# rayanirban/DiffSplitting

Measured on AMD Instinct MI355X. Metric: sampled images/sec (2000-step 128x128 SR3), higher is better.
Workload: dtype bf16; 1 GPU; sr_sr3_16_128: GaussianDiffusion.p_sample_loop, 16->128 SR3 UNet (97.8M params), T=2000 linear schedule; one step = UNet forward + posterior update of the batch; batch_per_gpu=16, global_batch=16, image=128x128x3, sample_steps=2000, parallelism=1 independent replicas, final RCCL all-gather, hipgraph=True, streams=1, noise=device Philox4x32-10, weights=random-init, seed 0

## Files before the change

diffsplitting_amd/csrc/dsx_conv_direct.hip:

```cpp
#include "dsx_conv_common.h"

namespace dsx {

template <typename DT>
__global__ __launch_bounds__(256) void k_conv_first(const ConvArgs a) {
  constexpr bool F32 = sizeof(DT) == 4;
  constexpr int ES = (int)sizeof(DT);
  constexpr int KSTEP = F32 ? 2 : 16;
  constexpr int NS16 = 4;
  __shared__ __attribute__((aligned(16))) unsigned char sm[18 * 18 * 7 * 4 + 64 * 4];
  DT* patch = (DT*)sm;
  int* kofft = (int*)(sm + 18 * 18 * 7 * 4);

  const int tid = threadIdx.x, lane = tid & 63;
  const int wave = __builtin_amdgcn_readfirstlane(tid >> 6);
  const int li = lane & 31, lh = lane >> 5;
  const int Cin = a.C0 + a.C1, K = 9 * Cin;
  const int tiles_x = a.Wo >> 4, tiles_y = a.Ho >> 4;
  const int t = blockIdx.x % (tiles_x * tiles_y), b = blockIdx.x / (tiles_x * tiles_y);
  const int ty = t / tiles_x, tx = t - ty * tiles_x;
  const int oy0 = ty * 16, ox0 = tx * 16;
  const int NBLK = (a.Cout + 31) >> 5;

  for (int e = tid; e < 18 * 18 * Cin; e += 256) {
// ... 37 lines not shown
#pragma unroll
  for (int mb = 0; mb < 2; ++mb)
#pragma unroll
    for (int nb = 0; nb < 2; ++nb)
#pragma unroll
      for (int r = 0; r < 16; ++r) acc[mb][nb][r] = 0.f;

#pragma unroll
  for (int mb = 0; mb < 2; ++mb) {
    const int m = (wave * 2 + mb) * 32 + li;
    const int base = ((m >> 4) * 18 + (m & 15)) * Cin;
    if constexpr (F32) {
      const int nsteps = (K + 1) >> 1;
      const float* wp = (const float*)a.wpack;
      for (int s = 0; s < nsteps; ++s) {
        const float pv = ((const float*)patch)[base + kofft[2 * s + lh]];
#pragma unroll
        for (int nb = 0; nb < 2; ++nb) {
          if (nb < NBLK) acc[mb][nb] = __builtin_amdgcn_mfma_f32_32x32x2f32(wp[(nb * 32 + s) * 64 + lane], pv, acc[mb][nb], 0, 0, 0);
        }
      }
    } else {
      const unsigned char* pb = (const unsigned char*)patch + base * 2;
#pragma unroll
      for (int s = 0; s < NS16; ++s) {
        unsigned w4[4];
#pragma unroll
        for (int q = 0; q < 4; ++q) {
          const unsigned lo = *(const unsigned short*)(pb + koff[s * 8 + 2 * q]);
          const unsigned hi = *(const unsigned short*)(pb + koff[s * 8 + 2 * q + 1]);
          w4[q] = lo | (hi << 16);
        }
        const f32x4_t px = __builtin_bit_cast(f32x4_t, make_uint4(w4[0], w4[1], w4[2], w4[3]));
#pragma unroll
        for (int nb = 0; nb < 2; ++nb)
          if (nb < NBLK) acc[mb][nb] = mfma_step<DT>(wf[nb * NS16 + s], px, acc[mb][nb]);
      }
    }
  }
  (void)KSTEP; (void)ES;

  const int okind = a.out_bf16;
#pragma unroll
  for (int nb = 0; nb < 2; ++nb) {
    const int nbase = nb * 32 + 16 * lh;
    if (nb >= NBLK) continue;
    float s1[16], s2[16];
#pragma unroll
    for (int r = 0; r < 16; ++r) { s1[r] = 0.f; s2[r] = 0.f; }
    const bool live = nbase < a.Cout;
#pragma unroll
    for (int mb = 0; mb < 2; ++mb) {
      const int m = (wave * 2 + mb) * 32 + li;
      const size_t opix = ((size_t)b * a.Ho + (oy0 + (m >> 4))) * a.Wo + (ox0 + (m & 15));
      float x[16], pv[16];
#pragma unroll
      for (int r = 0; r < 16; ++r) { x[r] = acc[mb][nb][r]; pv[r] = 0.f; }
      if (live) {
        if (a.bias) {
#pragma unroll
          for (int j = 0; j < 4; ++j) { const float4 tt = *(const float4*)(a.bias + nbase + 4 * j); pv[4 * j] = tt.x; pv[4 * j + 1] = tt.y; pv[4 * j + 2] = tt.z; pv[4 * j + 3] = tt.w; }
#pragma unroll
          for (int r = 0; r < 16; ++r) x[r] += pv[r];
        }
        store16<true>(a.out, opix * a.out_ld + nbase, x, okind, 16);
#pragma unroll
        for (int r = 0; r < 16; ++r) { const float d = x[r] - pv[r]; s1[r] += d; s2[r] += d * d; }
      }
    }
    if (a.stat_part != nullptr) {
      float w1 = row16_fold(s1, lane), w2 = row16_fold(s2, lane);
      w1 += __shfl_xor(w1, 16, 64);
      w2 += __shfl_xor(w2, 16, 64);
      const int nch = tiles_x * tiles_y * 4, chunk = t * 4 + wave;
      const int n = nbase + row16_fold_reg(li);
      if (li < 16 && n < a.Cout) {
        float* pp = a.stat_part + (((size_t)b * nch + chunk) * a.Cout + n) * 2;
        pp[0] = w1; pp[1] = w2;
      }
    }
  }
}

bool conv_first_applicable(int ks, int stride, const ConvArgs& a, bool gn) {
  const int C = a.C0 + a.C1;
  return ks == 3 && stride == 1 && !a.up && !gn && !a.swish && C >= 1 && C <= 7 && a.Cout >= 16 && a.Cout <= 64 &&
         (a.Cout & 15) == 0 && (a.Ho & 15) == 0 && (a.Wo & 15) == 0 && a.Ho == a.Hs && a.Wo == a.Ws && a.out_ld == a.Cout;
}
hipError_t launch_conv_first(int dtype, const ConvArgs& a, hipStream_t st) {
  const unsigned grid = (unsigned)(a.B * (a.Ho >> 4) * (a.Wo >> 4));
  if (dtype == 1) hipLaunchKernelGGL(k_conv_first<__bf16>, dim3(grid), dim3(256), 0, st, a);
  else if (dtype == 2) hipLaunchKernelGGL(k_conv_first<_Float16>, dim3(grid), dim3(256), 0, st, a);
  else hipLaunchKernelGGL(k_conv_first<float>, dim3(grid), dim3(256), 0, st, a);
  return hipGetLastError();
}

__global__ void k_conv_naive(const NaiveConvArgs na) {
  const ConvArgs& a = na.c;
  const long long total = (long long)a.B * a.Ho * a.Wo * a.Cout;
  const int C = a.C0 + a.C1;
  const int pad = na.ks / 2;
  const int Hi = a.up ? a.Hs * 2 : a.Hs, Wi = a.up ? a.Ws * 2 : a.Ws;
  for (long long idx = blockIdx.x * (long long)blockDim.x + threadIdx.x; idx < total;
       idx += (long long)gridDim.x * blockDim.x) {
    const int n = (int)(idx % a.Cout);
    long long p = idx / a.Cout;
    const int ox = (int)(p % a.Wo); p /= a.Wo;
    const int oy = (int)(p % a.Ho);
    const int b = (int)(p / a.Ho);
    float acc = 0.f;
    for (int dy = 0; dy < na.ks; ++dy) {
      const int iy = oy * na.stride + dy - pad;
      if (iy < 0 || iy >= Hi) continue;
      for (int dx = 0; dx < na.ks; ++dx) {
        const int ix = ox * na.stride + dx - pad;
        if (ix < 0 || ix >= Wi) continue;
        const int sy = a.up ? iy >> 1 : iy, sx = a.up ? ix >> 1 : ix;
        const size_t so = ((size_t)b * a.Hs + sy) * a.Ws + sx;
        const float* w = na.w + (((size_t)n * na.ks + dy) * na.ks + dx) * C;
        for (int c = 0; c < C; ++c) {
          float v = c < a.C0 ? act_load_kind(a.src0, so * a.C0 + c, a.act_bf16)
                             : act_load_kind(a.src1, so * a.C1 + (c - a.C0), a.act_bf16);
          if (a.gn_scale) v = v * a.gn_scale[(size_t)b * C + c] + a.gn_shift[(size_t)b * C + c];
          if (a.swish) v = swish_f(v);
          acc = fmaf(v, w[c], acc);
        }
      }
    }
    const size_t opix = ((size_t)b * a.Ho + oy) * a.Wo + ox;
    float v = acc + (a.bias ? a.bias[n] : 0.f);
    if (a.film) v += a.film[(size_t)b * a.film_bs + n];
    if (a.resid) v += act_load_kind(a.resid, opix * a.resid_ld + n, a.act_bf16);
    if (na.sigmoid_out) v = 1.0f / (1.0f + __expf(-v));
    act_store(a.out, opix * a.out_ld + n, v, a.out_bf16);
  }
}

hipError_t launch_conv_naive(const NaiveConvArgs& a, hipStream_t st) {
  const long long total = (long long)a.c.B * a.c.Ho * a.c.Wo * a.c.Cout;
  long long blocks = (total + 255) / 256;
  if (blocks > 8192) blocks = 8192;
  hipLaunchKernelGGL(k_conv_naive, dim3((unsigned)blocks), dim3(256), 0, st, a);
  return hipGetLastError();
}

}
```

diffsplitting_amd/csrc/dsx_kernels.h:

```cpp
#pragma once
#include <hip/hip_runtime.h>
#include <stdint.h>

namespace dsx {

struct PrefetchArgs {
  const void* base;
  unsigned slice_bytes;
  int nslices;
  unsigned* sink;
};
inline unsigned fastdiv_magic(unsigned d) { return d <= 1 ? 0u : (unsigned)((1ull << 32) / d) + 1u; }
#if defined(__HIPCC__)
__device__ __forceinline__ unsigned fastdiv(unsigned n, unsigned magic) { return magic ? __umulhi(n, magic) : n; }
struct PfAcc { unsigned v[4]; };
__device__ __forceinline__ PfAcc l2_prefetch(const PrefetchArgs& pf, unsigned lin_block, unsigned nblocks_total, int tid, int nthreads) {
  PfAcc acc = {{0u, 0u, 0u, 0u}};
  if (pf.base == nullptr || pf.nslices <= 0) return acc;
  const unsigned label = lin_block & 7u, j = lin_block >> 3, n8 = (nblocks_total + 7u) >> 3;
  const unsigned lines = pf.slice_bytes >> 7;
  const unsigned per = (lines + n8 - 1u) / n8, l0 = j * per;
  const unsigned l1 = l0 + per < lines ? l0 + per : lines;
  const int s0 = pf.nslices < 8 ? (int)(label % (unsigned)pf.nslices) : (int)label;
  const int sstep = pf.nslices < 8 ? pf.nslices : 8;
// ... 85 lines not shown
            ps[u] += ch == 0 ? a.count * p : 0.0;
          }
        }
      }
#pragma unroll
      for (int u = 0; u < 8; ++u) { s += ps[u]; q += pq[u]; }
    }
  };
  const int c_own = c_lo + tid;
  const bool own = tid < cpg;
  const float g_own = own ? a.gamma[c_own] : 0.f, b_own = own ? a.beta[c_own] : 0.f;
  if (n0 > 0) accumulate(a.part0, a.f32_0, n0, a.nchunk0, a.C0, c_lo, a.piv0);
  if (n1 > 0) accumulate(a.part1, a.f32_1, n1, a.nchunk1, a.C1, c_lo + n0 - a.C0, a.piv1);
#pragma unroll
  for (int o = 32; o > 0; o >>= 1) { s += __shfl_xor(s, o, 64); q += __shfl_xor(q, o, 64); }
  if constexpr (NW > 1) {
    if ((tid & 63) == 0) { red[2 * (tid >> 6)] = s; red[2 * (tid >> 6) + 1] = q; }
    __syncthreads();
    s = 0; q = 0;
#pragma unroll
    for (int w = 0; w < NW; ++w) { s += red[2 * w]; q += red[2 * w + 1]; }
  }
  const double n = a.count * cpg;
  const double mean = s / n;
  double var = q / n - mean * mean;
  if (var < 0) var = 0;
  const float rstd = (float)(1.0 / sqrt(var + (double)a.eps));
  const float meanf = (float)mean;
  if (own) {
    const float sc = rstd * g_own;
    a.scale[(size_t)b * C + c_own] = sc;
    a.shift[(size_t)b * C + c_own] = b_own - meanf * sc;
  }
  for (int c = c_lo + tid + NT; c < c_lo + cpg; c += NT) {
    const float sc = rstd * a.gamma[c];
    a.scale[(size_t)b * C + c] = sc;
    a.shift[(size_t)b * C + c] = a.beta[c] - meanf * sc;
  }
}
#endif

struct ConvArgs {
  const void* src0;
  const void* src1;
  int act_bf16;
  int out_bf16;
  int C0, C1;
  int B, Hs, Ws;
  int up;
  int Ho, Wo;
  const float* gn_scale;
  const float* gn_shift;
  int has_gn;
  int swish;
  int stage_mode;
  const void* wpack;
  const float* bias;
  const float* film;
  int film_bs;
  const void* resid;
  int resid_ld;
  void* out;
  int out_ld;
  int Cout;
  int nblocks;
  int kchunks;
  int tw_log2, th_log2, tb_log2;
  int tiles_x, tiles_y, m_tiles, n_tiles;
  int lds_row;
  int cpg;
  int ws_wg_per_n;
  int ws_cpg;
  int xcd_bands;
  int ws_map;
  int ws_nt_log2;
  int ws_per;
  int ws_adv_x, ws_adv_y, ws_adv_b;
  int ws_dpy, ws_dpx;
  unsigned mg_tiles_x, mg_per_img, mg_pw, mg_wpn, mg_per;
  int ws_bigdiv;
  float* stat_part;
  unsigned* handoff_timeouts;
  int ws_direct;
  unsigned long long* stamp;
  int stamp_block;
  int ablate;
  const void* gn_part0; int gn_nchunk0, gn_pf32_0;
  const void* gn_part1; int gn_nchunk1, gn_pf32_1;
  StatPivot gn_piv0, gn_piv1;
  const float* gn_gamma; const float* gn_beta;
  int gn_groups; float gn_eps;
  PrefetchArgs pf;
  int fin_on;
  GnFinArgs fin;
  int ksplit;
  int groups_per_split;
  long long slab_stride;
};

enum ConvTile { TILE_256x128 = 0, TILE_128x128, TILE_64x128, TILE_256x64, TILE_128x64, TILE_64x64, TILE_128x32, TILE_256x32, TILE_COUNT };
struct ConvTileInfo { int BM, BN, WM; bool fuses_stats; };
ConvTileInfo conv_tile_info(int tile, bool ws = false);
int conv_chunk_multiple(int ks);
constexpr int conv_lds_row(int ks, int stride, int tw_log2, int cpg) {
  const int pixb = 64 * cpg + 16;
  const int pw = ((1 << tw_log2) - 1) * stride + ks;
  int rb = (pw * pixb + 15) & ~15;
  if (ks == 1 || stride != 1) return rb;
  if (tw_log2 == 4) rb = (rb + 255) & ~255;
  else if (tw_log2 == 3) { rb = (rb + 127) & ~127; if (((rb >> 7) & 1) == 0) rb += 128; }
  return rb;
}
size_t conv_lds_bytes(int dtype, int tile, int ks, int stride, const ConvArgs& a);
hipError_t launch_conv(int dtype, int tile, int ks, int stride, const ConvArgs& a, hipStream_t st);
size_t conv_ws_lds_bytes(int dtype, int tile, int ks, const ConvArgs& a);
hipError_t launch_conv_ws(int dtype, int tile, int ks, const ConvArgs& a, hipStream_t st);
bool conv_img_applicable(int dtype, int ks, int stride, const ConvArgs& a, bool gn, int gn_groups);
hipError_t launch_conv_img(int dtype, int ks, const ConvArgs& a, hipStream_t st);
bool conv_first_applicable(int ks, int stride, const ConvArgs& a, bool gn);
hipError_t launch_conv_first(int dtype, const ConvArgs& a, hipStream_t st);
hipError_t conv_init();
hipError_t ops_init();

struct NaiveConvArgs {
  ConvArgs c;
  const float* w;
  int ks, stride;
  int sigmoid_out;
};
hipError_t launch_conv_naive(const NaiveConvArgs& a, hipStream_t st);

hipError_t launch_chan_stats(const void* x, int bf16, int B, int HW, int C, int nchunk, double* part,
                             hipStream_t st);
hipError_t launch_gn_finalize(const GnFinArgs& a, hipStream_t st);

struct TembArgs {
  int flavour;
  int B;
  int n_time;
  const float* time;
  const float* table;
  const int* step_ctr;
  int per_sample;
  int inner;
  const float* freq;
  const float* w1; const float* b1;
  const float* w2; const float* b2;
  const float* wf; const float* bf;
  int F;
  float* film;
};
hipError_t launch_temb(const TembArgs& a, hipStream_t st);

struct SplitKReduceArgs {
  const float* slab; int nsplit; long long slab_stride;
  long long M; int N; int HW;
  const float* bias; const float* film; int film_bs;
  const void* resid; int resid_ld;
  void* out;
  int act_bf16;
  float* stat_part;
};
hipError_t launch_splitk_reduce(const SplitKReduceArgs& a, hipStream_t st);

struct AttnArgs {
  const void* q; const void* k; const void* v; int ld;
  void* out; int ldo;
  int storage;
  int B, L, C;
  float div, inv_div;
};
bool attn_supported(int C, int L);
hipError_t launch_attn(const AttnArgs& a, bool col_split, hipStream_t st);

hipError_t launch_nchw_slice_to_nhwc(const float* src, void* dst, int dst_bf16, int B, int C, int ctot, int coff,
                                     int HW, hipStream_t st);
hipError_t launch_nhwc_to_nchw(const float* src, float* dst, int B, int C, int H, int W, hipStream_t st);

constexpr int kUpdateCols = 7;
struct UpdateArgs {
  float* x;
  void* x_act;
  int x_act_kind;
  const float* net;
  float* x0_hist;
  int use_noise;
  const unsigned long long* loop_params;
  const float* tab;
  int n_steps;
  const int* step_ctr;
  int predict_eps, clip;
  int per_sample;
  int B, C, H, W;
  const unsigned long long* sample_ids;
};
hipError_t launch_update(const UpdateArgs& a, hipStream_t st);
constexpr int kStreamRows = 32;
struct StreamIds { unsigned long long subseq[kStreamRows]; };
template <class F>
static inline hipError_t each_stream_chunk(int B, const uint64_t* ids, uint64_t draw, F&& f) {
  for (int b0 = 0; b0 < B; b0 += kStreamRows) {
    StreamIds s{};
// ... 323 lines not shown
```

diffsplitting_amd/csrc/dsx_plan.cpp:

```cpp
#include "dsx_rt.h"

static std::vector<int> tile_order(const char* e, const std::vector<int>& dflt) {
  if (!*e) return dflt;
  std::vector<int> v;
  for (const char* p = e; *p;) {
    v.push_back(atoi(p));
    while (*p && *p != ',') ++p;
    if (*p == ',') ++p;
  }
  return v;
}

PlanKnobs dsx::read_plan_knobs() {
  PlanKnobs k;
  static const struct { const char* name; int PlanKnobs::*field; } ints[] = {
      {"DSX_FIRST", &PlanKnobs::first}, {"DSX_IMG", &PlanKnobs::img}, {"DSX_WS", &PlanKnobs::ws},
      {"DSX_WS_1X1", &PlanKnobs::ws_1x1}, {"DSX_WS_MIN_GRID", &PlanKnobs::ws_min_grid}, {"DSX_WS_G2", &PlanKnobs::ws_g2},
      {"DSX_WS_G2_MIN64", &PlanKnobs::ws_g2_min64}, {"DSX_WS_G2_MIN128", &PlanKnobs::ws_g2_min128},
      {"DSX_WS_G4_MIN64", &PlanKnobs::ws_g4_min64}, {"DSX_WS_C4", &PlanKnobs::ws_c4},
      {"DSX_WS_C4_MIN", &PlanKnobs::ws_c4_min}, {"DSX_WS_DIRECT", &PlanKnobs::ws_direct}, {"DSX_WS_MAP3", &PlanKnobs::ws_map3},
      {"DSX_XCD_BANDS", &PlanKnobs::xcd_bands}, {"DSX_HOST_FIN", &PlanKnobs::host_fin},
      {"DSX_PREFETCH", &PlanKnobs::prefetch}, {"DSX_PREFETCH_WS", &PlanKnobs::prefetch_ws},
      {"DSX_FUSE_STATS", &PlanKnobs::fuse_stats}, {"DSX_NARROW_G2", &PlanKnobs::narrow_g2},
      {"DSX_MIN_GRID", &PlanKnobs::min_grid}, {"DSX_SPLITK", &PlanKnobs::splitk}, {"DSX_ATTN_CS", &PlanKnobs::attn_cs},
#ifdef DSX_DIAG
      {"DSX_ABLATE", &PlanKnobs::ablate},
#endif
  };
  static const struct { const char* name; std::vector<int> PlanKnobs::*field; } lists[] = {
      {"DSX_TILES_WIDE", &PlanKnobs::tiles_wide}, {"DSX_TILES_NARROW", &PlanKnobs::tiles_narrow},
      {"DSX_TILES_SLIM", &PlanKnobs::tiles_slim}, {"DSX_TILES_WIDE_SPLIT", &PlanKnobs::tiles_wide_split},
      {"DSX_TILES_NARROW_SPLIT", &PlanKnobs::tiles_narrow_split}, {"DSX_TILES_NARROW_G2", &PlanKnobs::tiles_narrow_g2},
      {"DSX_TILES_WS_WIDE", &PlanKnobs::tiles_ws_wide}, {"DSX_TILES_WS_WIDE_1X1", &PlanKnobs::tiles_ws_wide_1x1},
      {"DSX_TILES_WS_WIDE_1X1_RAW", &PlanKnobs::tiles_ws_wide_1x1_raw}, {"DSX_TILES_WS_NARROW", &PlanKnobs::tiles_ws_narrow},
  };
  for (const auto& e : ints)
    if (const char* v = getenv(e.name)) k.*e.field = atoi(v);
  for (const auto& e : lists)
    if (const char* v = getenv(e.name)) k.*e.field = tile_order(v, k.*e.field);
  const char* impl = getenv("DSX_CONV_IMPL");
  k.conv_naive = impl && !strcmp(impl, "naive");
  if (const char* path = getenv("DSX_PLAN_DUMP")) k.plan_dump = path;
  if (const char* se = getenv("DSX_STAMP_OP")) {
    const char* comma = strchr(se, ',');
    k.stamp_op = atoi(se);
    k.stamp_block = comma ? atoi(comma + 1) : 0;
  }
  return k;
}

hipError_t dsx::launch_op(const PlanOp& o, hipStream_t st) {
  switch (o.launcher) {
    case L_CONV_FIRST: return launch_conv_first(o.dtype, o.args.conv, st);
    case L_CONV_IMG: return launch_conv_img(o.dtype, o.ks, o.args.conv, st);
    case L_CONV_WS: return launch_conv_ws(o.dtype, o.tile, o.ks, o.args.conv, st);
    case L_CONV_MFMA: return launch_conv(o.dtype, o.tile, o.ks, o.stride, o.args.conv, st);
    case L_SPLITK_REDUCE: return launch_splitk_reduce(o.args.reduce, st);
    case L_CONV_NAIVE: return launch_conv_naive(o.args.naive, st);
    case L_CHAN_STATS: {
      const ChanStatsArgs& c = o.args.stats;
      return launch_chan_stats(c.x, c.xbf, c.B, c.HW, c.C, c.nchunk, c.part, st);
    }
    case L_GN_FINALIZE: return launch_gn_finalize(o.args.fin, st);
    case L_ATTN: return launch_attn(o.args.attn, o.col_split != 0, st);
  }
  return hipErrorInvalidValue;
}

static int dump_plan(const dsx_exec* ex) {
  static const struct { const char* name; size_t bytes; } L[] = {
      {"conv_first", sizeof(ConvArgs)}, {"conv_img", sizeof(ConvArgs)}, {"conv_ws", sizeof(ConvArgs)},
      {"conv_mfma", sizeof(ConvArgs)}, {"splitk_reduce", sizeof(SplitKReduceArgs)}, {"conv_naive", sizeof(NaiveConvArgs)},
      {"chan_stats", sizeof(ChanStatsArgs)}, {"gn_finalize", sizeof(GnFinArgs)}, {"attn", sizeof(AttnArgs)}};
  FILE* f = fopen(ex->knobs.plan_dump.c_str(), "w");
  if (!f) return fail(DSX_ERR_INVALID, "DSX_PLAN_DUMP: cannot write %s", ex->knobs.plan_dump.c_str());
  for (size_t i = 0; i < ex->ops.size(); ++i) {
    const PlanOp& o = ex->ops[i];
    const char* name = (o.launcher == L_GN_FINALIZE && gn_finalize_is_wide(o.args.fin)) ? "gn_finalize_wide" : L[o.launcher].name;
    fprintf(f, "%zu kind=%d desc=\"%s\" flops=%.17g bytes=%.17g launcher=%s dtype=%d tile=%d ks=%d stride=%d col_split=%d args=",
            i, o.kind, o.desc.c_str(), o.flops, o.bytes, name, o.dtype, o.tile, o.ks, o.stride, o.col_split);
    const unsigned char* p = (const unsigned char*)&o.args;
    for (size_t b = 0; b < L[o.launcher].bytes; ++b) fprintf(f, "%02x", p[b]);
    fputc('\n', f);
  }
  fclose(f);
  return DSX_OK;
}

static int add_op(dsx_exec* ex, int kind, const std::string& desc, double flops, double bytes, Launcher launcher) {
  PlanOp op;
  op.kind = kind; op.desc = desc; op.flops = flops; op.bytes = bytes; op.launcher = launcher;
  ex->ops.push_back(op);
  return (int)ex->ops.size() - 1;
}
static std::string fmt(const char* f, ...) {
  char buf[256];
  va_list ap;
  va_start(ap, f);
  vsnprintf(buf, sizeof buf, f, ap);
  va_end(ap);
  return buf;
}

static char* ws_alloc(dsx_exec* ex, size_t bytes) {
  size_t off = (ex->ws_used + 255) & ~(size_t)255;
  ex->ws_used = off + bytes;
  if (ex->sizing) return nullptr;
// ... 135 lines not shown
    if (wpn > a.m_tiles) wpn = (a.m_tiles + unit - 1) / unit * unit;
  }
  return wpn;
}

static void decide_ws_chunks(const PlanKnobs& k, int dtype, int ks, int tile, ConvArgs& a) {
  auto take = [&](bool wanted, int cpg) {
    ConvArgs t = a;
    t.ws_cpg = cpg; t.lds_row = conv_lds_row(ks, 1, a.tw_log2, cpg);
    if (wanted && conv_ws_lds_bytes(dtype, tile, ks, t) != 0) { a.ws_cpg = cpg; a.lds_row = t.lds_row; }
  };
  if (ks == 3) {
    const int min_chunks = conv_tile_info(tile).BM == 64 ? k.ws_g2_min64 : k.ws_g2_min128;
    take(k.ws_g2 && a.kchunks >= min_chunks, 2);
    take(k.ws_g2 && a.kchunks >= k.ws_g4_min64, 4);
  }
  if (ks == 1) take(k.ws_c4 && a.kchunks >= k.ws_c4_min, 4);
  if (ks == 1 && k.ws_direct && !a.has_gn && !a.swish) {
    ConvArgs t = a;
    t.ws_direct = 1;
    if (conv_ws_lds_bytes(dtype, tile, ks, t) != 0) a.ws_direct = 1;
  }
}

static int decide_ws_startup(const PlanKnobs& k, int ks, ConvArgs& w) {
  w.xcd_bands = k.xcd_bands;
  w.ws_wg_per_n = ws_wg_per_n(w);
  const bool map3 = k.ws_map3 && ks == 1 && w.n_tiles >= 2 && w.n_tiles <= 32;
  if (map3) {
    int wpn3 = std::max(8, (256 / w.n_tiles) / 8 * 8);
    if (wpn3 > w.m_tiles) wpn3 = (w.m_tiles + 7) / 8 * 8;
    w.ws_wg_per_n = wpn3;
  }
  const int NT = w.n_tiles, wpn = w.ws_wg_per_n, per_img = w.tiles_x * w.tiles_y;
  w.ws_map = map3 ? 3 : ((NT <= 8 && 8 % NT == 0 && wpn % (8 / NT) == 0) ? 0 : ((NT % 8) == 0 ? 1 : 2));
  w.ws_nt_log2 = NT <= 8 ? ilog2(NT) : 0;
  w.ws_per = map3 ? NT : (NT >> 3);
  w.ws_adv_x = wpn % w.tiles_x; w.ws_adv_y = (wpn / w.tiles_x) % w.tiles_y; w.ws_adv_b = wpn / per_img;
  const int PW = ((1 << w.tw_log2) - 1) + ks;
  const int upg = 4 * (w.ws_cpg ? w.ws_cpg : conv_chunk_multiple(ks));
  const int pstep = 256 / upg;
  w.ws_dpy = pstep / PW; w.ws_dpx = pstep - w.ws_dpy * PW;
  w.mg_tiles_x = fastdiv_magic((unsigned)w.tiles_x); w.mg_per_img = fastdiv_magic((unsigned)per_img);
  w.mg_pw = fastdiv_magic((unsigned)PW); w.mg_wpn = fastdiv_magic((unsigned)wpn);
  w.mg_per = fastdiv_magic((unsigned)std::max(1, w.ws_per));
  w.ws_bigdiv = ((long long)w.m_tiles + wpn >= 65536 || w.tiles_x >= 65536 || per_img >= 65536) ? 1 : 0;
  auto exact = [](unsigned d, unsigned magic, unsigned nmax) {
    for (unsigned n = 0; n <= nmax; ++n) {
      const unsigned q = magic ? (unsigned)(((unsigned long long)n * magic) >> 32) : n;
      if (q != n / d) return false;
    }
    return true;
  };
  const unsigned grid = (unsigned)(NT * wpn);
  const unsigned nt_max = w.ws_bigdiv ? 0u : (unsigned)(w.m_tiles + wpn);
  if (!exact((unsigned)w.tiles_x, w.mg_tiles_x, grid) || !exact((unsigned)per_img, w.mg_per_img, grid) ||
      !exact((unsigned)PW, w.mg_pw, 255u) || !exact((unsigned)wpn, w.mg_wpn, std::max(grid, nt_max)) ||
      !exact((unsigned)std::max(1, w.ws_per), w.mg_per, grid >> 3))
    return fail(DSX_ERR_INVALID, "planner: fastdiv magic not exact for conv %dx%d @%dx%d", ks, ks, w.Ho, w.Wo);
  return DSX_OK;
}

static int decide_conv(const PlanKnobs& k, int dtype, int norm_groups, const ConvShape& s, ConvChoice& ch) {
  ch = ConvChoice{};
  ch.tile = -1;
  ConvArgs& a = ch.geo;
  a.C0 = s.C0; a.C1 = s.C1;
  a.B = s.B; a.Hs = s.Hs; a.Ws = s.Ws; a.up = s.up ? 1 : 0;
  a.Ho = s.Ho; a.Wo = s.Wo;
  a.swish = s.swish ? 1 : 0;
  a.has_gn = s.has_gn ? 1 : 0;
  a.act_bf16 = dtype;
  a.out_bf16 = s.out_st;
  {
    const int gw = conv_chunk_multiple(s.ks) * (dtype != 0 ? 32 : 16);
    const int um = dtype != 0 ? 7 : 3;
    a.stage_mode = ((a.C0 & um) || (a.C1 & um)) ? 2 : ((a.C1 == 0 || a.C0 % gw == 0) ? 0 : 1);
  }
  a.resid_ld = s.resid_ld; a.out_ld = s.out_ld; a.Cout = s.Cout;
  a.nblocks = s.nblocks; a.kchunks = s.kchunks;
  const int ks = s.ks, stride = s.stride;
  if (!k.conv_naive && k.first && !s.has_film && !s.has_resid && conv_first_applicable(ks, stride, a, s.has_gn)) {
    ch.kernel = CONV_FIRST;
    if (s.want_stats) { ch.stats = STATS_EPILOGUE; ch.stat_nchunk = (a.Ho >> 4) * (a.Wo >> 4) * 4; ch.pivot = PIVOT_BIAS; }
    return DSX_OK;
  }
  if (!k.conv_naive && k.img && !(s.has_resid && (s.resid_ld & 3)) &&
      conv_img_applicable(dtype, ks, stride, a, s.has_gn, norm_groups)) {
    ch.kernel = CONV_IMG;
    ch.gn_in_kernel = s.has_gn;
    if (s.want_stats) { ch.stats = STATS_EPILOGUE; ch.stat_nchunk = 1; }
    return DSX_OK;
  }
  const bool ws_allowed = k.ws && (ks != 1 || k.ws_1x1) && stride == 1 && a.stage_mode == 0;
  if (k.conv_naive || !decide_tile(k, dtype, ks, stride, ws_allowed, a, ch.tile)) {
    if (!s.has_naive)
      return fail(DSX_ERR_INVALID, "no MFMA tile fits conv %dx%d (%dx%d out, B=%d); set DSX_CONV_IMPL=naive", ks, ks,
                  a.Ho, a.Wo, a.B);
    ch.kernel = CONV_NAIVE;
    return DSX_OK;
  }
  const int tile = ch.tile;
  const bool use_ws = ws_allowed && a.cpg != 2 && a.ksplit == 1 && conv_ws_lds_bytes(dtype, tile, ks, a) != 0;
  ch.kernel = a.ksplit > 1 ? CONV_SPLITK : (use_ws ? CONV_WS : (a.cpg == 2 ? CONV_MFMA_G2 : CONV_MFMA));
  if (use_ws) decide_ws_chunks(k, dtype, ks, tile, a);
  const ConvTileInfo ti = conv_tile_info(tile, use_ws);
  if (k.fuse_stats && s.want_stats && ti.fuses_stats &&
      a.ksplit == 1 && a.tb_log2 == 0 && (a.Cout & 15) == 0 && a.out_ld == a.Cout && (a.resid_ld & 7) == 0) {
    ch.stats = STATS_EPILOGUE;
    ch.stat_nchunk = a.tiles_x * a.tiles_y * ti.WM;
  }
  if (a.ksplit > 1 && k.fuse_stats && s.want_stats && a.Cout % 64 == 0 && a.out_ld == a.Cout && (a.Ho * a.Wo) % 16 == 0) {
    ch.stats = STATS_REDUCE;
    ch.stat_nchunk = a.Ho * a.Wo / 16;
    ch.pivot = PIVOT_BIAS_FILM;
  }
  ch.hosts_fin = s.may_host_fin && k.host_fin && use_ws;
  return use_ws ? decide_ws_startup(k, ks, a) : DSX_OK;
}

struct ConvSpec {
  const ConvW* w;
  Tensor x0, x1;
  bool up = false;
  int stride = 1;
  const GnW* gn = nullptr;
  bool has_resid = false;
  bool host_fin = false;
  bool swish = false;
  int film_off = -1;
  const void* resid = nullptr; int resid_ld = 0;
  Tensor out;
  bool want_stats = false;
  bool bias_in_film = false;
};

static bool reserve_stats(dsx_exec* ex, const Tensor& t) {
  StatInfo& si = ex->stats[t.id];
  if (si.planned) return false;
  int nchunk = std::max(1, 512 / ex->B);
  nchunk = std::min(nchunk, std::max(1, t.H * t.W / 16));
  nchunk = std::min(nchunk, 64);
  si.nchunk = nchunk;
  si.part = ws_alloc(ex, (size_t)ex->B * nchunk * t.C * 2 * sizeof(double));
  si.planned = true;
  si.f32 = false;
  return true;
}
static void emit_stats(dsx_exec* ex, const Tensor& t) {
  const StatInfo& si = ex->stats[t.id];
  const int HW = t.H * t.W;
  const int i = add_op(ex, DSX_OP_GN_STATS, fmt("gn_stats C=%d @%dx%d", t.C, t.H, t.W), 0.0,
                       (t.st ? 2.0 : 4.0) * ex->B * HW * t.C, L_CHAN_STATS);
  ChanStatsArgs& c = ex->ops[i].args.stats;
  c.x = t.p; c.xbf = t.st; c.B = ex->B; c.HW = HW; c.C = t.C; c.nchunk = si.nchunk; c.part = (double*)si.part;
}

static float* plan_fused_stats(dsx_exec* ex, const Tensor& t, int nchunk, int C) {
  StatInfo& si = ex->stats[t.id];
  si.nchunk = nchunk;
  si.part = ws_alloc(ex, (size_t)ex->B * nchunk * C * 2 * sizeof(float));
  si.planned = true;
  si.f32 = true;
  return (float*)si.part;
}

// ... 385 lines not shown
```

diffsplitting_amd/csrc/dsx_rt.h:

```cpp
#pragma once
#include <hip/hip_runtime.h>

#include <algorithm>
#include <cmath>
#include <cstdarg>
#include <cstdio>
#include <cstdlib>
#include <cstring>
#include <memory>
#include <string>
#include <utility>
#include <vector>

#include "../../include/dsx.h"
#include "dsx_kernels.h"

using namespace dsx;

namespace dsx {

int fail(int code, const char* fmt, ...);
#define HIP_TRY(expr)                                                                     \
  do {                                                                                    \
    hipError_t e__ = (expr);                                                              \
// ... 11 lines not shown
  void reset() { if (p) (void)hipFree(p); p = nullptr; }
  template <class T> T* as() const { return (T*)p; }
  hipError_t alloc(size_t bytes) {
    reset();
    const hipError_t e = hipMalloc(&p, bytes);
    if (e != hipSuccess) p = nullptr;
    return e;
  }
  hipError_t upload(const void* host, size_t bytes) {
    const hipError_t e = alloc(bytes);
    return e != hipSuccess ? e : hipMemcpy(p, host, bytes, hipMemcpyHostToDevice);
  }
};
struct PinnedBuf {
  void* p = nullptr;
  PinnedBuf() = default;
  PinnedBuf(PinnedBuf&& o) noexcept : p(o.p) { o.p = nullptr; }
  PinnedBuf& operator=(PinnedBuf&& o) noexcept { std::swap(p, o.p); return *this; }
  ~PinnedBuf() { reset(); }
  void reset() { if (p) (void)hipHostFree(p); p = nullptr; }
  template <class T> T* as() const { return (T*)p; }
  hipError_t alloc(size_t bytes) {
    reset();
    const hipError_t e = hipHostMalloc(&p, bytes, hipHostMallocDefault);
    if (e != hipSuccess) p = nullptr;
    return e;
  }
};
struct Event {
  hipEvent_t e = nullptr;
  Event() = default;
  Event(Event&& o) noexcept : e(o.e) { o.e = nullptr; }
  Event& operator=(Event&& o) noexcept { std::swap(e, o.e); return *this; }
  ~Event() { reset(); }
  void reset() { if (e) (void)hipEventDestroy(e); e = nullptr; }
  hipError_t create(unsigned flags = hipEventDefault) { reset(); return hipEventCreateWithFlags(&e, flags); }
};
struct Stream {
  hipStream_t s = nullptr;
  Stream() = default;
  Stream(Stream&& o) noexcept : s(o.s) { o.s = nullptr; }
  Stream& operator=(Stream&& o) noexcept { std::swap(s, o.s); return *this; }
  ~Stream() { reset(); }
  void reset() { if (s) (void)hipStreamDestroy(s); s = nullptr; }
  hipError_t create(unsigned flags) { reset(); return hipStreamCreateWithFlags(&s, flags); }
};
struct Graph {
  hipGraph_t graph = nullptr;
  hipGraphExec_t exec = nullptr;
  Graph() = default;
  Graph(Graph&& o) noexcept : graph(o.graph), exec(o.exec) { o.graph = nullptr; o.exec = nullptr; }
  Graph& operator=(Graph&& o) noexcept { std::swap(graph, o.graph); std::swap(exec, o.exec); return *this; }
  ~Graph() { reset(); }
  void reset() {
    if (exec) (void)hipGraphExecDestroy(exec);
    if (graph) (void)hipGraphDestroy(graph);
    exec = nullptr; graph = nullptr;
  }
};

struct PlanKnobs {
  bool conv_naive = false;
  int first = 1;
  int img = 1;
  int ws = 1;
  int ws_1x1 = 1;
  int ws_min_grid = 224;
  int ws_g2 = 1;
  int ws_g2_min64 = 12;
  int ws_g2_min128 = 4;
  int ws_g4_min64 = 16;
  int ws_c4 = 1;
  int ws_c4_min = 8;
  int ws_direct = 1;
  int ws_map3 = 1;
  int xcd_bands = 1;
  int host_fin = 1;
  int prefetch = 1;
  int prefetch_ws = 1;
  int fuse_stats = 1;
  int narrow_g2 = 1;
  int min_grid = 512;
  int splitk = 1;
  int attn_cs = 2;
  int stamp_op = -1;
  int stamp_block = 0;
  std::string plan_dump;
  int ablate = 0;
  std::vector<int> tiles_wide{TILE_128x128, TILE_64x128, TILE_64x64};
  std::vector<int> tiles_narrow{TILE_64x64, TILE_128x64};
  std::vector<int> tiles_slim{TILE_128x32, TILE_64x64, TILE_128x64};
  std::vector<int> tiles_wide_split{TILE_64x128, TILE_128x128, TILE_64x64};
  std::vector<int> tiles_narrow_split{TILE_64x64, TILE_128x64};
  std::vector<int> tiles_narrow_g2{TILE_256x32, TILE_128x32};
  std::vector<int> tiles_ws_wide{TILE_128x128, TILE_64x128};
  std::vector<int> tiles_ws_wide_1x1{TILE_128x128, TILE_64x128};
  std::vector<int> tiles_ws_wide_1x1_raw{TILE_64x128, TILE_128x128};
  std::vector<int> tiles_ws_narrow{TILE_256x64, TILE_128x64, TILE_64x64};
};

struct Param {
  std::string name;
  std::vector<int64_t> shape;
  std::vector<float> host;
  bool set = false;
  int64_t numel() const {
    int64_t n = 1;
    for (auto s : shape) n *= s;
    return n;
  }
};

struct ConvW {
  int pw = -1, pb = -1;
  int cin = 0, cout = 0, ks = 1;
  int kchunks = 0, nblocks = 0;
  void* pack = nullptr;
  void* pack_first = nullptr;
  float* bias = nullptr;
  float* naive = nullptr;
};
struct GnW {
  int pg = -1, pb = -1;
  int C = 0;
  float* gamma = nullptr;
  float* beta = nullptr;
};
struct LinW {
  int pw = -1, pb = -1;
  int in = 0, out = 0;
};

struct Module {
  int kind;
  int section;
  int cin = 0, cout = 0, skip = 0;
  bool attn = false;
  ConvW conv;
  GnW gn1, gn2, gna;
  ConvW conv1, conv2, res, qkv, out;
  bool has_res = false;
  LinW film;
  int film_off = -1;
};

}

struct dsx_model {
  dsx_unet_cfg cfg;
  std::vector<Param> params;
  std::vector<Module> mods;
  int p_invfreq = -1;
  LinW t1, t2;
  std::vector<float> freq;
  bool freq_set = false;
  int F = 0;
  bool finalized = false;
  int dtype = 0;
  DevBuf arena;
  size_t arena_bytes = 0;
  float *d_freq = nullptr, *d_w1 = nullptr, *d_b1 = nullptr, *d_w2 = nullptr, *d_b2 = nullptr;
  float *d_wf = nullptr, *d_bf = nullptr;
  bool want_naive = false;
};

namespace dsx {
// ... 81 lines not shown
```

Baseline: 2.982 images/s.

## Add persistent double-buffered streaming variant of first conv kernel

Adds a persistent version of the first-layer 3x3 conv that loops over 16x16 tiles with a grid capped at two workgroups per CU. Each tile's input patch is prefetched into registers and committed to a second LDS buffer while the current tile computes. Weights and bias are loaded once per workgroup. Patch addresses use precomputed offsets and border bitmasks, with paired 32-bit LDS reads when the channel count is even. It is enabled by default through a new planner knob, which adds kernel complexity, and the first conv is a small part of the UNet step.

```diff
diff --git a/diffsplitting_amd/csrc/dsx_conv_direct.hip b/diffsplitting_amd/csrc/dsx_conv_direct.hip
--- a/diffsplitting_amd/csrc/dsx_conv_direct.hip
+++ b/diffsplitting_amd/csrc/dsx_conv_direct.hip
@@ -143,12 +143,247 @@
   }
 }
 
+template <typename DT>
+__global__ __launch_bounds__(256, CONV_FIRST_STREAM_WG_PER_CU) void k_conv_first_stream(const ConvArgs a) {
+  constexpr bool F32 = sizeof(DT) == 4;
+  constexpr int NS16 = 4;
+  constexpr int PATCH = 18 * 18 * 7 * 4 + 16;
+  constexpr int NE = 9;
+  using RT = typename std::conditional<F32, float, unsigned short>::type;
+  __shared__ __attribute__((aligned(16))) unsigned char sm[2 * PATCH + 2 * 64 * 4 + (F32 ? 2 * 32 * 64 * 4 : 0)];
+  float* biasl = (float*)(sm + 2 * PATCH);
+  int* kofft = (int*)(sm + 2 * PATCH + 64 * 4);
+  float* wl = (float*)(sm + 2 * PATCH + 2 * 64 * 4);
+
+  const int tid = threadIdx.x, lane = tid & 63;
+  const int wave = __builtin_amdgcn_readfirstlane(tid >> 6);
+  const int li = lane & 31, lh = lane >> 5;
+  const int Cin = a.C0 + a.C1, K = 9 * Cin;
+  const int tiles_x = a.Wo >> 4, per_img = tiles_x * (a.Ho >> 4);
+  const int ntiles = a.B * per_img;
+  const int NBLK = (a.Cout + 31) >> 5;
+  const int total = 18 * 18 * Cin;
+  const bool pairs = !F32 && (Cin & 1) == 0;
+  const unsigned mC = (65536u + Cin - 1) / Cin;
+
+  int rel[NE];
+  unsigned eb_lo = 0, eb_hi = 0;
+#pragma unroll
+  for (int j = 0; j < NE; ++j) {
+    const int e = tid + 256 * j;
+    const int pp = (int)(((unsigned)e * mC) >> 16), c = e - pp * Cin, py = pp / 18, px = pp - py * 18;
+    const bool s1 = c >= a.C0;
+    rel[j] = ((py - 1) * a.Ws + (px - 1)) * (s1 ? a.C1 : a.C0) + (s1 ? c - a.C0 : c);
+    const unsigned bits = (py == 0 ? 1u : 0u) | (py == 17 ? 2u : 0u) | (px == 0 ? 4u : 0u) | (px == 17 ? 8u : 0u) | (s1 ? 16u : 0u);
+    if (e >= total) rel[j] = 0;
+    if (j < 6) eb_lo |= (e < total ? bits : 0u) << (5 * j);
+    else eb_hi |= (e < total ? bits : 0u) << (5 * (j - 6));
+  }
+  auto ebits = [&](int j) { return (j < 6 ? eb_lo >> (5 * j) : eb_hi >> (5 * (j - 6))) & 31u; };
+
+  struct Tile { int b, tl, oy0, ox0; };
+  auto decode = [&](int t) {
+    Tile T;
+    T.b = t / per_img; T.tl = t - T.b * per_img;
+    const int ty = T.tl / tiles_x;
+    T.oy0 = ty * 16; T.ox0 = (T.tl - ty * tiles_x) * 16;
+    return T;
+  };
+  auto request = [&](const Tile& T, RT (&v)[NE], unsigned& okm) __attribute__((always_inline)) {
+    const size_t pix = ((size_t)T.b * a.Hs + T.oy0) * a.Ws + T.ox0;
+    const RT* p0 = (const RT*)a.src0 + pix * a.C0;
+    const RT* p1 = (const RT*)a.src1 + pix * a.C1;
+    const unsigned tf = (T.oy0 == 0 ? 1u : 0u) | (T.oy0 + 16 == a.Hs ? 2u : 0u) | (T.ox0 == 0 ? 4u : 0u) | (T.ox0 + 16 == a.Ws ? 8u : 0u);
+    okm = 0;
+#pragma unroll
+    for (int j = 0; j < NE; ++j) {
+      const unsigned bits = ebits(j);
+      const bool ok = (bits & tf) == 0;
+      const RT* p = (bits & 16u) ? p1 : p0;
+      v[j] = p[ok ? rel[j] : 0];
+      okm |= (ok ? 1u : 0u) << j;
+    }
+  };
+  auto commit = [&](int buf, const RT (&v)[NE], unsigned okm) __attribute__((always_inline)) {
+    RT* patch = (RT*)(sm + buf * PATCH);
+#pragma unroll
+    for (int j = 0; j < NE; ++j) {
+      const int e = tid + 256 * j;
+      patch[e < total ? e : total] = ((okm >> j) & 1u) ? v[j] : (RT)0;
+    }
+  };
+
+  uint4 wf[F32 ? 1 : 2 * NS16];
+  if constexpr (!F32) {
+#pragma unroll
+    for (int nb = 0; nb < 2; ++nb)
+#pragma unroll
+      for (int s = 0; s < NS16; ++s)
+        wf[nb * NS16 + s] = nb < NBLK ? ((const uint4*)a.wpack)[(nb * NS16 + s) * 64 + lane] : make_uint4(0u, 0u, 0u, 0u);
+  } else {
+    for (int i = tid; i < NBLK * 32 * 64; i += 256) wl[i] = ((const float*)a.wpack)[i];
+  }
+  if (tid < 64) biasl[tid] = (a.bias != nullptr && tid < a.Cout) ? a.bias[tid] : 0.f;
+
+  RT pv_next[NE];
+  unsigned ok_next = 0;
+#pragma unroll
+  for (int j = 0; j < NE; ++j) pv_next[j] = (RT)0;
+  int t = blockIdx.x;
+  Tile T = decode(t);
+  request(T, pv_next, ok_next);
+
+  if (F32 && tid < 64) {
+    const int k = tid < K ? tid : 0;
+    const int tap = (int)(((unsigned)k * mC) >> 16), c = k - tap * Cin;
+    kofft[tid] = ((tap / 3) * 18 + (tap % 3)) * Cin + c;
+  }
+  unsigned koff[F32 ? 1 : NS16 * 4];
+  if constexpr (!F32) {
+#pragma unroll
+    for (int s = 0; s < NS16; ++s)
+#pragma unroll
+      for (int j = 0; j < 8; ++j) {
+        int k = 16 * s + 8 * lh + j;
+        if (k >= K) k = 0;
+        const int tap = (int)(((unsigned)k * mC) >> 16), c = k - tap * Cin;
+        const unsigned off = (unsigned)((((tap / 3) * 18 + (tap % 3)) * Cin + c) * 2);
+        if (j & 1) koff[s * 4 + (j >> 1)] |= pairs ? 0u : off << 16;
+        else koff[s * 4 + (j >> 1)] = off;
+      }
+  }
+  int base[2];
+#pragma unroll
+  for (int mb = 0; mb < 2; ++mb) {
+    const int m = (wave * 2 + mb) * 32 + li;
+    base[mb] = ((m >> 4) * 18 + (m & 15)) * Cin;
+  }
+  commit(0, pv_next, ok_next);
+  wait_vmcnt<0>();
+  __syncthreads();
+
+  const int okind = a.out_bf16;
+#pragma clang loop unroll(disable)
+  for (int cur = 0; t < ntiles; t += gridDim.x, cur ^= 1) {
+    const int tn = t + (int)gridDim.x;
+    const bool more = tn < ntiles;
+    const Tile Tn = more ? decode(tn) : T;
+    if (more) request(Tn, pv_next, ok_next);
+
+    const unsigned char* patch = sm + cur * PATCH;
+    f32x16 acc[2][2];
+#pragma unroll
+    for (int mb = 0; mb < 2; ++mb)
+#pragma unroll
+      for (int nb = 0; nb < 2; ++nb)
+#pragma unroll
+        for (int r = 0; r < 16; ++r) acc[mb][nb][r] = 0.f;
+
+#pragma unroll
+    for (int mb = 0; mb < 2; ++mb) {
+      if constexpr (F32) {
+        const int nsteps = (K + 1) >> 1;
+        for (int s = 0; s < nsteps; ++s) {
+          const float pv = ((const float*)patch)[base[mb] + kofft[2 * s + lh]];
+#pragma unroll
+          for (int nb = 0; nb < 2; ++nb) {
+            if (nb < NBLK) acc[mb][nb] = __builtin_amdgcn_mfma_f32_32x32x2f32(wl[(nb * 32 + s) * 64 + lane], pv, acc[mb][nb], 0, 0, 0);
+          }
+        }
+      } else {
+        const unsigned char* pb = patch + base[mb] * 2;
+        auto steps = [&](auto PAIRS) __attribute__((always_inline)) {
+#pragma unroll
+          for (int s = 0; s < NS16; ++s) {
+            unsigned w4[4];
+#pragma unroll
+            for (int q = 0; q < 4; ++q) {
+              if constexpr (decltype(PAIRS)::value) {
+                w4[q] = *(const unsigned*)(pb + koff[s * 4 + q]);
+              } else {
+                const unsigned lo = *(const unsigned short*)(pb + (koff[s * 4 + q] & 0xffffu));
+                const unsigned hi = *(const unsigned short*)(pb + (koff[s * 4 + q] >> 16));
+                w4[q] = lo | (hi << 16);
+              }
+            }
+            const f32x4_t px = __builtin_bit_cast(f32x4_t, make_uint4(w4[0], w4[1], w4[2], w4[3]));
+#pragma unroll
+            for (int nb = 0; nb < 2; ++nb)
+              acc[mb][nb] = mfma_step<DT>(wf[nb * NS16 + s], px, acc[mb][nb]);
+          }
+        };
+        if (pairs) steps(std::true_type{});
+        else steps(std::false_type{});
+      }
+    }
+
+    if (more) {
+      commit(cur ^ 1, pv_next, ok_next);
+      __syncthreads();
+    }
+
+#pragma unroll
+    for (int nb = 0; nb < 2; ++nb) {
+      const int nbase = nb * 32 + 16 * lh;
+      if (nb >= NBLK) continue;
+      float s1[16], s2[16];
+#pragma unroll
+      for (int r = 0; r < 16; ++r) { s1[r] = 0.f; s2[r] = 0.f; }
+      const bool live = nbase < a.Cout;
+#pragma unroll
+      for (int mb = 0; mb < 2; ++mb) {
+        const int m = (wave * 2 + mb) * 32 + li;
+        const size_t opix = ((size_t)T.b * a.Ho + (T.oy0 + (m >> 4))) * a.Wo + (T.ox0 + (m & 15));
+        float x[16], pv[16];
+#pragma unroll
+        for (int r = 0; r < 16; ++r) { x[r] = acc[mb][nb][r]; pv[r] = 0.f; }
+        if (live) {
+          if (a.bias) {
+#pragma unroll
+            for (int j = 0; j < 4; ++j) { const float4 tt = *(const float4*)(biasl + nbase + 4 * j); pv[4 * j] = tt.x; pv[4 * j + 1] = tt.y; pv[4 * j + 2] = tt.z; pv[4 * j + 3] = tt.w; }
+#pragma unroll
+            for (int r = 0; r < 16; ++r) x[r] += pv[r];
+          }
+          store16<true>(a.out, opix * a.out_ld + nbase, x, okind, 16);
+#pragma unroll
+          for (int r = 0; r < 16; ++r) { const float d = x[r] - pv[r]; s1[r] += d; s2[r] += d * d; }
+        }
+      }
+      if (a.stat_part != nullptr) {
+        float w1 = row16_fold(s1, lane), w2 = row16_fold(s2, lane);
+        w1 += __shfl_xor(w1, 16, 64);
+        w2 += __shfl_xor(w2, 16, 64);
+        const int nch = per_img * 4, chunk = T.tl * 4 + wave;
+        const int n = nbase + row16_fold_reg(li);
+        if (li < 16 && n < a.Cout) {
+          float* pp = a.stat_part + (((size_t)T.b * nch + chunk) * a.Cout + n) * 2;
+          pp[0] = w1; pp[1] = w2;
+        }
+      }
+    }
+
+    T = Tn;
+  }
+}
+
 bool conv_first_applicable(int ks, int stride, const ConvArgs& a, bool gn) {
   const int C = a.C0 + a.C1;
   return ks == 3 && stride == 1 && !a.up && !gn && !a.swish && C >= 1 && C <= 7 && a.Cout >= 16 && a.Cout <= 64 &&
          (a.Cout & 15) == 0 && (a.Ho & 15) == 0 && (a.Wo & 15) == 0 && a.Ho == a.Hs && a.Wo == a.Ws && a.out_ld == a.Cout;
 }
+int conv_first_stream_grid(const ConvArgs& a, int forced) {
+  const int tiles = a.B * (a.Ho >> 4) * (a.Wo >> 4);
+  const int want = forced > 0 ? forced : 256 * CONV_FIRST_STREAM_WG_PER_CU;
+  return want < tiles ? want : tiles;
+}
 hipError_t launch_conv_first(int dtype, const ConvArgs& a, hipStream_t st) {
+  if (a.first_grid > 0) {
+    const unsigned grid = (unsigned)a.first_grid;
+    if (dtype == 1) hipLaunchKernelGGL(k_conv_first_stream<__bf16>, dim3(grid), dim3(256), 0, st, a);
+    else if (dtype == 2) hipLaunchKernelGGL(k_conv_first_stream<_Float16>, dim3(grid), dim3(256), 0, st, a);
+    else hipLaunchKernelGGL(k_conv_first_stream<float>, dim3(grid), dim3(256), 0, st, a);
+    return hipGetLastError();
+  }
   const unsigned grid = (unsigned)(a.B * (a.Ho >> 4) * (a.Wo >> 4));
   if (dtype == 1) hipLaunchKernelGGL(k_conv_first<__bf16>, dim3(grid), dim3(256), 0, st, a);
   else if (dtype == 2) hipLaunchKernelGGL(k_conv_first<_Float16>, dim3(grid), dim3(256), 0, st, a);
diff --git a/diffsplitting_amd/csrc/dsx_kernels.h b/diffsplitting_amd/csrc/dsx_kernels.h
--- a/diffsplitting_amd/csrc/dsx_kernels.h
+++ b/diffsplitting_amd/csrc/dsx_kernels.h
@@ -191,6 +191,7 @@
   float* stat_part;
   unsigned* handoff_timeouts;
   int ws_direct;
+  int first_grid;
   unsigned long long* stamp;
   int stamp_block;
   int ablate;
@@ -227,6 +228,8 @@
 bool conv_img_applicable(int dtype, int ks, int stride, const ConvArgs& a, bool gn, int gn_groups);
 hipError_t launch_conv_img(int dtype, int ks, const ConvArgs& a, hipStream_t st);
 bool conv_first_applicable(int ks, int stride, const ConvArgs& a, bool gn);
+constexpr int CONV_FIRST_STREAM_WG_PER_CU = 2;
+int conv_first_stream_grid(const ConvArgs& a, int forced);
 hipError_t launch_conv_first(int dtype, const ConvArgs& a, hipStream_t st);
 hipError_t conv_init();
 hipError_t ops_init();
diff --git a/diffsplitting_amd/csrc/dsx_plan.cpp b/diffsplitting_amd/csrc/dsx_plan.cpp
--- a/diffsplitting_amd/csrc/dsx_plan.cpp
+++ b/diffsplitting_amd/csrc/dsx_plan.cpp
@@ -23,6 +23,7 @@
       {"DSX_PREFETCH", &PlanKnobs::prefetch}, {"DSX_PREFETCH_WS", &PlanKnobs::prefetch_ws},
       {"DSX_FUSE_STATS", &PlanKnobs::fuse_stats}, {"DSX_NARROW_G2", &PlanKnobs::narrow_g2},
       {"DSX_MIN_GRID", &PlanKnobs::min_grid}, {"DSX_SPLITK", &PlanKnobs::splitk}, {"DSX_ATTN_CS", &PlanKnobs::attn_cs},
+      {"DSX_EDGE_STREAM", &PlanKnobs::edge_stream}, {"DSX_EDGE_GRID", &PlanKnobs::edge_grid},
 #ifdef DSX_DIAG
       {"DSX_ABLATE", &PlanKnobs::ablate},
 #endif
@@ -324,6 +325,7 @@
   const int ks = s.ks, stride = s.stride;
   if (!k.conv_naive && k.first && !s.has_film && !s.has_resid && conv_first_applicable(ks, stride, a, s.has_gn)) {
     ch.kernel = CONV_FIRST;
+    a.first_grid = k.edge_stream ? conv_first_stream_grid(a, k.edge_grid) : 0;
     if (s.want_stats) { ch.stats = STATS_EPILOGUE; ch.stat_nchunk = (a.Ho >> 4) * (a.Wo >> 4) * 4; ch.pivot = PIVOT_BIAS; }
     return DSX_OK;
   }
diff --git a/diffsplitting_amd/csrc/dsx_rt.h b/diffsplitting_amd/csrc/dsx_rt.h
--- a/diffsplitting_amd/csrc/dsx_rt.h
+++ b/diffsplitting_amd/csrc/dsx_rt.h
@@ -117,6 +117,8 @@
   int narrow_g2 = 1;
   int min_grid = 512;
   int splitk = 1;
+  int edge_stream = 1;
+  int edge_grid = 0;
   int attn_cs = 2;
   int stamp_op = -1;
   int stamp_block = 0;
```

New measurement: 2.987 images/s, median of 2. No clear change (+0.2%).
